# als244/ResNet

Measured on AMD Instinct MI355X. Metric: images/sec ResNet-50 fp32 224x224 batch256, higher is better.
Workload: dtype f32

## Files before the change

resnet_amd/csrc/kernels_bn.hip:

```cpp
#include "mi_common.hpp"
#include "mi_device.h"

#define BN_SPLIT_MAX 64

struct Wel { float n, mean, m2; };
__device__ __forceinline__ Wel wel_merge(Wel a, Wel b) {
    Wel r;
    r.n = a.n + b.n;
    if (r.n == 0.f) { r.mean = 0.f; r.m2 = 0.f; return r; }
    const float d = b.mean - a.mean, f = b.n / r.n;
    r.mean = a.mean + d * f;
    r.m2 = a.m2 + b.m2 + d * d * a.n * f;
    return r;
}
__device__ __forceinline__ Wel wel_wave(Wel w) {
#pragma unroll
    for (int o = 32; o > 0; o >>= 1) {
        Wel b;
        b.n = __shfl_xor(w.n, o, 64); b.mean = __shfl_xor(w.mean, o, 64); b.m2 = __shfl_xor(w.m2, o, 64);
        w = wel_merge(w, b);
    }
    return w;
}
__device__ __forceinline__ void wel_add4(Wel &w, float a, float b, float c, float d) {
// ... 64 lines not shown
    }
    w = wel_wave(w);
    __shared__ Wel sh[4];
    const int lane = threadIdx.x & 63, wv = threadIdx.x >> 6;
    if (lane == 0) sh[wv] = w;
    __syncthreads();
    if (threadIdx.x == 0) {
        Wel r = sh[0];
        for (int i = 1; i < (int)(blockDim.x >> 6); i++) r = wel_merge(r, sh[i]);
        float *o = partial + ((size_t)c * BN_SPLIT_MAX + split) * 3;
        o[0] = r.n; o[1] = r.mean; o[2] = r.m2;
    }
}

__global__ void __launch_bounds__(256)
bn_parts_merge_kernel(const float *__restrict__ parts, int np, int C, float *__restrict__ partial) {
    const int cx = threadIdx.x & 63, sg = threadIdx.x >> 6;
    const int c = blockIdx.x * 64 + cx;
    const int chunk = (np + gridDim.y - 1) / gridDim.y;
    const int p0 = blockIdx.y * chunk, p1 = min(np, p0 + chunk);
    const size_t plane = (size_t)np * C;
    Wel w = {0.f, 0.f, 0.f};
    if (c < C) {
        int p = p0 + sg;
        for (; p + 7 * 4 < p1; p += 8 * 4) {
            Wel b[8];
#pragma unroll
            for (int u = 0; u < 8; u++) {
                const size_t o = (size_t)(p + 4 * u) * C + c;
                b[u].n = parts[o]; b[u].mean = parts[plane + o]; b[u].m2 = parts[2 * plane + o];
            }
#pragma unroll
            for (int u = 0; u < 8; u++) w = wel_merge(w, b[u]);
        }
        for (; p < p1; p += 4) {
            const size_t o = (size_t)p * C + c;
            Wel b = {parts[o], parts[plane + o], parts[2 * plane + o]};
            w = wel_merge(w, b);
        }
    }
    __shared__ Wel sh[4][64];
    sh[sg][cx] = w;
    __syncthreads();
    if (sg == 0 && c < C) {
        Wel r = sh[0][cx];
        for (int i = 1; i < 4; i++) r = wel_merge(r, sh[i][cx]);
        float *o = partial + ((size_t)c * BN_SPLIT_MAX + blockIdx.y) * 3;
        o[0] = r.n; o[1] = r.mean; o[2] = r.m2;
    }
}

__global__ void __launch_bounds__(256)
bn_finalize_kernel(const float *__restrict__ partial, int nsplit, int C, float *__restrict__ means, float *__restrict__ vars) {
    const int c = blockIdx.x * 4 + (threadIdx.x >> 6), lane = threadIdx.x & 63;
    if (c >= C) return;
    const float *p = partial + (size_t)c * BN_SPLIT_MAX * 3;
    Wel w = {0.f, 0.f, 0.f};
    if (lane < nsplit) { w.n = p[lane * 3]; w.mean = p[lane * 3 + 1]; w.m2 = p[lane * 3 + 2]; }
    w = wel_wave(w);
    if (lane == 0) { means[c] = w.mean; vars[c] = w.m2 / w.n; }
}
// ... 169 lines not shown
    }
    s1 = wave_sum(s1); s2 = wave_sum(s2);
    __shared__ float sh[8];
    const int lane = threadIdx.x & 63, wv = threadIdx.x >> 6;
    if (lane == 0) { sh[wv * 2] = s1; sh[wv * 2 + 1] = s2; }
    __syncthreads();
    if (threadIdx.x == 0) {
        float a = 0.f, bsum = 0.f;
        for (int i = 0; i < (int)(blockDim.x >> 6); i++) { a += sh[i * 2]; bsum += sh[i * 2 + 1]; }
        float *o = partial + ((size_t)c * BN_SPLIT_MAX + split) * 3;
        o[0] = a; o[1] = bsum;
    }
}

__global__ void __launch_bounds__(256)
bn_bwd_parts_merge_kernel(const float *__restrict__ parts, int np, int C, const float *__restrict__ vars, float eps, float *__restrict__ partial) {
    const int cx = threadIdx.x & 63, sg = threadIdx.x >> 6;
    const int c = blockIdx.x * 64 + cx;
    const int chunk = (np + gridDim.y - 1) / gridDim.y;
    const int p0 = blockIdx.y * chunk, p1 = min(np, p0 + chunk);
    const size_t plane = (size_t)np * C;
    float a1 = 0.f, a2 = 0.f;
    if (c < C) {
        int p = p0 + sg;
        for (; p + 7 * 4 < p1; p += 8 * 4) {
            float u1[8], u2[8];
#pragma unroll
            for (int u = 0; u < 8; u++) {
                const size_t o = (size_t)(p + 4 * u) * C + c;
                u1[u] = parts[o]; u2[u] = parts[plane + o];
            }
#pragma unroll
            for (int u = 0; u < 8; u++) { a1 += u1[u]; a2 += u2[u]; }
        }
        for (; p < p1; p += 4) {
            const size_t o = (size_t)p * C + c;
            a1 += parts[o]; a2 += parts[plane + o];
        }
    }
    __shared__ float sh[2][4][64];
    sh[0][sg][cx] = a1; sh[1][sg][cx] = a2;
    __syncthreads();
    if (sg == 0 && c < C) {
        const float s1 = (sh[0][0][cx] + sh[0][1][cx]) + (sh[0][2][cx] + sh[0][3][cx]);
        const float s2 = (sh[1][0][cx] + sh[1][1][cx]) + (sh[1][2][cx] + sh[1][3][cx]);
        float *o = partial + ((size_t)c * BN_SPLIT_MAX + blockIdx.y) * 3;
        o[0] = s1; o[1] = s2 / sqrtf(vars[c] + eps);
    }
}

__global__ void __launch_bounds__(256)
bn_bwd_finalize_kernel(float *__restrict__ partial, int nsplit, int C, float *__restrict__ dgamma, float *__restrict__ dbeta) {
    const int c = blockIdx.x * 4 + (threadIdx.x >> 6), lane = threadIdx.x & 63;
    if (c >= C) return;
    const float *p = partial + (size_t)c * BN_SPLIT_MAX * 3;
    float s1 = 0.f, s2 = 0.f;
    if (lane < nsplit) { s1 = p[lane * 3]; s2 = p[lane * 3 + 1]; }
    s1 = wave_sum(s1); s2 = wave_sum(s2);
    if (lane == 0) { dbeta[c] = s1; dgamma[c] = s2; }
}

template <int MASK, typename TX, typename TA, int V, bool STR>
// ... 236 lines not shown
    if ((xhat_out || norm_out) && !(x_dt == MID_F32 && a_dt == MID_F32)) { mi_record_error("mid_bn_fwd_t", "full-store tensors exist in fp32 only"); return -2; }
    if (bn_size_ok("mid_bn_fwd_t", N, C, P)) return -2;
    hipStream_t st = (hipStream_t)s;
    const double xb = (double)N * C * P * dt_bytes(x_dt), ab = (double)N * C * P * dt_bytes(a_dt);
    if (!parts || parts->nparts <= 0) {
        const int ns = bn_nsplit(N, C);
        mi_prof_begin(st, MI_FAM_BN, 0.0, 2 * xb + ab * (residual ? 2 : 1));
        if (bn_stats_launch(st, ws, x, x_dt, N, C, P, ns)) return -1;
        hipLaunchKernelGGL(bn_finalize_kernel, dim3(mi_cdiv(C, 4)), dim3(256), 0, st, ws, ns, C, means, vars);
        MI_LAUNCH_CHECK("bn_finalize_kernel");
    } else {
        int G = parts->nparts / 64;
        if (G < 1) G = 1;
        if (G > BN_SPLIT_MAX) G = BN_SPLIT_MAX;
        mi_prof_begin(st, MI_FAM_BN, 0.0, xb + ab * (residual ? 2 : 1));
        hipLaunchKernelGGL(bn_parts_merge_kernel, dim3(mi_cdiv(C, 64), G), dim3(256), 0, st, parts->buf, parts->nparts, C, ws);
        MI_LAUNCH_CHECK("bn_parts_merge_kernel");
        hipLaunchKernelGGL(bn_finalize_kernel, dim3(mi_cdiv(C, 4)), dim3(256), 0, st, ws, G, C, means, vars);
        MI_LAUNCH_CHECK("bn_finalize_kernel");
    }
    if (g_bn_sync.comm && g_bn_sync.world > 1 - g_bn_sync.force) {
        const float iw = 1.0f / (float)g_bn_sync.world;
        float *tmp = g_bn_sync.tmp;
        if (C > g_bn_sync.tmp_floats / 2) { mi_record_error("sync BN", "scratch too small"); return -3; }
        (void)hipMemcpyAsync(tmp, means, sizeof(float) * C, hipMemcpyDeviceToDevice, st);
        if (mid_rccl_allreduce_sum(g_bn_sync.comm, tmp, (size_t)C, (mid_stream)st)) return -1;
        hipLaunchKernelGGL(bn_sync_k2, dim3(mi_cdiv(C, 256)), dim3(256), 0, st, tmp, means, vars, tmp + C, C, iw);
        if (mid_rccl_allreduce_sum(g_bn_sync.comm, tmp + C, (size_t)C, (mid_stream)st)) return -1;
        hipLaunchKernelGGL(bn_sync_k3, dim3(mi_cdiv(C, 256)), dim3(256), 0, st, tmp + C, vars, C, iw);
        MI_LAUNCH_CHECK("bn_sync");
    }
    const int rc = bn_fwd_apply(st, x, x_dt, gamma, beta, residual, means, vars, y, a_dt, xhat_out, norm_out, N, C, P, eps, relu, ycl, Hcl);
    mi_prof_end(st);
    return rc;
// ... 12 lines not shown
}

static int bn_bwd_impl(hipStream_t st, float *ws, const void *x, int x_dt, const float *gamma, const float *beta, const float *means,
                       const float *vars, const void *dy, const void *mask_src, void *gated_out, int a_dt, void *dx, float *dgamma,
                       float *dbeta, int N, int C, int P, float eps, int mask_mode, const mid_bn_bwd_parts *bparts = nullptr) {
    if (!bn_pair_ok(x_dt, a_dt)) { mi_record_error("mid_bn_bwd", "unsupported storage types"); return -2; }
    if (bn_size_ok("mid_bn_bwd", N, C, P)) return -2;
    int ns = bn_nsplit(N, C);
    dim3 grid(C, ns), block(256);
    if (mask_mode >= 2 && !mask_src) { mi_record_error("mid_bn_bwd", "mask_src missing"); return -2; }
    if (mask_mode == 3 && !gated_out) { mi_record_error("mid_bn_bwd_gate", "gated_out missing"); return -2; }
    const double xb = (double)N * C * P * dt_bytes(x_dt), ab = (double)N * C * P * dt_bytes(a_dt);
    mi_prof_begin(st, MI_FAM_BN, 0.0, bparts ? 2 * xb + ab : 3 * xb + ab * (mask_mode >= 2 ? 4 : 2));
    const int vec = bn_vec(x_dt, a_dt, P);
    const FastDiv fdPV = make_fastdiv(P / vec);
    if (bparts) {
        ns = bparts->nparts >= 64 * 8 ? 64 : bparts->nparts >= 64 ? 8 : 1;
        hipLaunchKernelGGL(bn_bwd_parts_merge_kernel, dim3(mi_cdiv(C, 64), ns), dim3(256), 0, st, bparts->buf, bparts->nparts, C, vars, eps, ws);
        MI_LAUNCH_CHECK("bn_bwd_parts_merge_kernel");
    } else {
#define BWD_REDUCE_M(M_, TX, TA, V)                                                                                         \
    hipLaunchKernelGGL((bn_bwd_reduce_kernel<M_, TX, TA, V>), grid, block, 0, st, (const TX *)x, (const TA *)dy, (const TA *)mask_src, \
                       gamma, beta, means, vars, ws, (TA *)gated_out, N, C, P, eps, fdPV)
#define BWD_R0(TX, TA, V) BWD_REDUCE_M(0, TX, TA, V)
#define BWD_R1(TX, TA, V) BWD_REDUCE_M(1, TX, TA, V)
#define BWD_R2(TX, TA, V) BWD_REDUCE_M(2, TX, TA, V)
#define BWD_R3(TX, TA, V) BWD_REDUCE_M(3, TX, TA, V)
    if (mask_mode == 0) BN_DISPATCH(BWD_R0);
    else if (mask_mode == 1) BN_DISPATCH(BWD_R1);
    else if (mask_mode == 2) BN_DISPATCH(BWD_R2);
    else BN_DISPATCH(BWD_R3);
#undef BWD_R0
#undef BWD_R1
#undef BWD_R2
#undef BWD_R3
#undef BWD_REDUCE_M
    MI_LAUNCH_CHECK("bn_bwd_reduce_kernel");
    }
    hipLaunchKernelGGL(bn_bwd_finalize_kernel, dim3(mi_cdiv(C, 4)), dim3(256), 0, st, ws, ns, C, dgamma, dbeta);
    MI_LAUNCH_CHECK("bn_bwd_finalize_kernel");
    const size_t total = (size_t)N * C * P;
    const FastDiv fdP = make_fastdiv(P), fdC = make_fastdiv(C);
    float inv_m = 1.0f / (float)((size_t)N * P);
    const float *dg_apply = dgamma, *db_apply = dbeta;
    const bool sync = g_bn_sync.comm && g_bn_sync.world > 1 - g_bn_sync.force;
    if (sync) {
        if (2 * C > g_bn_sync.tmp_floats) { mi_record_error("sync BN", "scratch too small"); return -3; }
        float *tmp = g_bn_sync.tmp;
        hipLaunchKernelGGL(bn_sync_pack, dim3(mi_cdiv(C, 256)), dim3(256), 0, st, dgamma, dbeta, tmp, C);
        if (mid_rccl_allreduce_sum(g_bn_sync.comm, tmp, (size_t)2 * C, (mid_stream)st)) return -1;
        dg_apply = tmp; db_apply = tmp + C;
        inv_m = 1.0f / ((float)g_bn_sync.world * (float)((size_t)N * P));
    }
    const void *dy_apply = mask_mode == 3 ? gated_out : dy;
    const char *apply_name;
// ... 57 lines not shown
```

resnet_amd/csrc/kernels_gemm.hip:

```cpp
#include "mi_common.hpp"
#include "mi_device.h"

typedef float f32x16 __attribute__((ext_vector_type(16)));

struct GemmArgs {
    int M, N, K;
    long a_sm, a_sk, a_sb;
    long b_sk, b_sn, b_sb;
    long c_sm, c_sn, c_sb;
    int P;
    FastDiv fdP;
    int klen;
    long c_split;
};

enum { BATCH_NONE = 0, BATCH_N = 1, BATCH_K = 2 };

#define G_BK 32
#define G_LDK 129
#define G_LDN 132

typedef float gf4 __attribute__((ext_vector_type(4)));

template <int BM, int BATCH, bool A_KC, bool B_KC, bool VA, bool VB>
__global__ void __launch_bounds__(256)
gemm_mfma_kernel(const float *__restrict__ A, const float *__restrict__ B, float *__restrict__ C,
                 const float *__restrict__ addend, const GemmArgs g) {
    constexpr int BN = 128;
    constexpr int WM = 64, WN = (BM == 128) ? 64 : 32;
    constexpr int TM = WM / 32, TN = WN / 32;
    constexpr int LDA = A_KC ? G_LDK : G_LDN, LDB = B_KC ? G_LDK : G_LDN;
    constexpr int AV = BM * G_BK / 1024, BV = BN * G_BK / 1024;
    constexpr int AE = BM * G_BK / 256, BE = BN * G_BK / 256;
    __shared__ __attribute__((aligned(16))) float As[G_BK * LDA];
    __shared__ __attribute__((aligned(16))) float Bs[G_BK * LDB];
    const int tid = threadIdx.x, lane = tid & 63;
    const int wave = __builtin_amdgcn_readfirstlane(tid >> 6);
    const int wm = (BM == 128) ? (wave >> 1) : 0, wn = (BM == 128) ? (wave & 1) : wave;
    const int m0 = blockIdx.y * BM, n0 = blockIdx.x * BN;
    const int kbeg = blockIdx.z * g.klen, kend = min(g.K, kbeg + g.klen);

    f32x16 acc[TM][TN];
#pragma unroll
    for (int i = 0; i < TM; i++)
#pragma unroll
        for (int j = 0; j < TN; j++)
#pragma unroll
            for (int r = 0; r < 16; r++) acc[i][j][r] = 0.f;

    constexpr int NA = VA ? AV : AE, NB = VB ? BV : BE;
    int ai[NA], ak[NA], bj[NB], bk[NB];
    long aoff[NA], boff[NB];
#pragma unroll
    for (int q = 0; q < NA; q++) {
        if (VA) {
            if (A_KC) { ak[q] = (tid & 7) * 4; ai[q] = (tid >> 3) + 32 * q; }
            else { ai[q] = (tid & (BM / 4 - 1)) * 4; ak[q] = tid / (BM / 4) + (1024 / BM) * q; }
        } else {
            if (A_KC) { ak[q] = tid & 31; ai[q] = (tid >> 5) + 8 * q; }
            else { ai[q] = tid % BM; ak[q] = tid / BM + (256 / BM) * q; }
        }
        aoff[q] = (long)(m0 + ai[q]) * g.a_sm;
    }
#pragma unroll
    for (int q = 0; q < NB; q++) {
        if (VB) {
            if (B_KC) { bk[q] = (tid & 7) * 4; bj[q] = (tid >> 3) + 32 * q; }
            else { bj[q] = (tid & 31) * 4; bk[q] = (tid >> 5) + 8 * q; }
        } else {
            if (B_KC) { bk[q] = tid & 31; bj[q] = (tid >> 5) + 8 * q; }
            else { bj[q] = tid & 127; bk[q] = (tid >> 7) + 2 * q; }
        }
        const int col = min(n0 + bj[q], g.N - 1);
        if (BATCH == BATCH_N) { const uint32_t n = fd_div((uint32_t)col, g.fdP); boff[q] = (long)n * g.b_sb + (col - (long)n * g.P); }
        else boff[q] = (long)col * g.b_sn;
    }
    auto koff_a = [&](int kk) -> long {
        if (BATCH == BATCH_K) { const uint32_t n = fd_div((uint32_t)kk, g.fdP); return (long)n * g.a_sb + (kk - (long)n * g.P); }
        return (long)kk * g.a_sk;
    };
    auto koff_b = [&](int kk) -> long {
        if (BATCH == BATCH_K) { const uint32_t n = fd_div((uint32_t)kk, g.fdP); return (long)n * g.b_sb + (kk - (long)n * g.P); }
        return (long)kk * g.b_sk;
    };

    gf4 ra4[VA ? AV : 1], rb4[VB ? BV : 1];
// ... 86 lines not shown
            for (int r = 0; r < 16; r++) {
                const int row = m0 + wm * WM + i * 32 + (r & 3) + 8 * (r >> 2) + 4 * (lane >> 5);
                if (row < g.M) {
                    const long o = coff + (long)row * g.c_sm;
                    float v = acc[i][j][r];
                    if (addend) v += ad[r];
                    Cz[o] = v;
                }
            }
        }
    }
}

template <int BATCH, bool A_KC, bool B_KC>
static int launch_gemm(hipStream_t st, const float *A, const float *B, float *C, const float *addend, GemmArgs g,
                       int splits, bool va, bool vb) {
    g.fdP = make_fastdiv(g.P > 0 ? g.P : 1);
    if (splits < 1) splits = 1;
    int klen = mi_cdiv(g.K, splits);
    klen = mi_cdiv(klen, G_BK) * G_BK;
    g.klen = klen;
    splits = mi_cdiv(g.K, klen);
    const int bm = g.M <= 64 ? 64 : 128;
    dim3 grid(mi_cdiv(g.N, 128), mi_cdiv(g.M, bm), splits), block(256);
    mi_prof_begin(st, MI_FAM_GEMM, 2.0 * (double)g.M * g.N * g.K,
                  4.0 * ((double)g.M * g.K + (double)g.K * g.N + (double)g.M * g.N * (addend ? 2 : 1)));
    if (((uintptr_t)A & 15) || ((uintptr_t)B & 15)) va = vb = false;
#define GL(BM_, VA_, VB_) hipLaunchKernelGGL((gemm_mfma_kernel<BM_, BATCH, A_KC, B_KC, VA_, VB_>), grid, block, 0, st, A, B, C, addend, g)
    if (bm == 64) { if (va && vb) GL(64, true, true); else if (va) GL(64, true, false); else GL(64, false, false); }
    else { if (va && vb) GL(128, true, true); else if (va) GL(128, true, false); else GL(128, false, false); }
#undef GL
    mi_prof_end(st);
    MI_LAUNCH_CHECK("gemm_mfma_kernel");
    return splits;
}

int mi_launch_split_reduce(hipStream_t st, const float *part, float *out, long n, int splits, size_t stride);

extern "C" int mi_conv1x1_fwd(mid_stream s, const float *x, const float *w, float *y, int N, int C, int P, int K) {
    hipStream_t st = (hipStream_t)s;
    GemmArgs g = {};
    g.M = K; g.N = N * P; g.K = C; g.P = P;
    g.a_sm = C; g.a_sk = 1;
    g.b_sk = P; g.b_sb = (long)C * P;
    g.c_sm = P; g.c_sb = (long)K * P;
    return launch_gemm<BATCH_N, true, false>(st, w, x, y, nullptr, g, 1, C % 4 == 0, P % 4 == 0) > 0 ? 0 : -1;
}
extern "C" int mi_conv1x1_dgrad(mid_stream s, const float *w, const float *dy, float *dx, const float *addend, int N, int C,
                                int P, int K) {
    hipStream_t st = (hipStream_t)s;
    GemmArgs g = {};
    g.M = C; g.N = N * P; g.K = K; g.P = P;
    g.a_sm = 1; g.a_sk = C;
    g.b_sk = P; g.b_sb = (long)K * P;
    g.c_sm = P; g.c_sb = (long)C * P;
    return launch_gemm<BATCH_N, false, false>(st, w, dy, dx, addend, g, 1, C % 4 == 0, P % 4 == 0) > 0 ? 0 : -1;
}
static int wgrad1x1_splits(int N, int C, int P, int K) {
    const int tiles = mi_cdiv(C, 128) * mi_cdiv(K, K <= 64 ? 64 : 128);
    int splits = mi_cdiv(1024, tiles);
    const long kd = (long)N * P;
    const int maxs = (int)(kd / 256 > 0 ? kd / 256 : 1);
    if (splits > maxs) splits = maxs;
    if (splits < 1) splits = 1;
    return splits;
}
extern "C" size_t mi_conv1x1_wgrad_part_floats(int N, int C, int P, int K) {
    return (size_t)wgrad1x1_splits(N, C, P, K) * K * C;
}
extern "C" int mi_conv1x1_wgrad(mid_stream s, mid_workspace *ws, const float *x, const float *dy, float *dw, int N, int C, int P,
                                int K) {
    hipStream_t st = (hipStream_t)s;
    GemmArgs g = {};
    g.M = K; g.N = C; g.K = N * P; g.P = P;
    g.a_sm = P; g.a_sb = (long)K * P;
    g.b_sn = P; g.b_sb = (long)C * P;
    g.c_sm = C; g.c_sn = 1;
    g.c_split = (long)K * C;
    int splits = wgrad1x1_splits(N, C, P, K);
    if (splits > 1 && (!ws || ws->part_floats < (size_t)splits * K * C)) {
        mi_record_error("mi_conv1x1_wgrad", "workspace too small");
        return -3;
    }
    float *out = splits > 1 ? ws->part : dw;
    const int used = launch_gemm<BATCH_K, true, true>(st, dy, x, out, nullptr, g, splits, P % 4 == 0, P % 4 == 0);
    if (used < 0) return -1;
    if (splits > 1) return mi_launch_split_reduce(st, out, dw, (long)K * C, used, (size_t)K * C);
    return 0;
}

extern "C" {
int mid_gemm_nn(mid_stream s, const float *A, const float *B, float *out, int m, int k, int n) {
    GemmArgs g = {};
    g.M = m; g.N = n; g.K = k; g.P = 1;
    g.a_sm = k; g.a_sk = 1; g.b_sk = n; g.b_sn = 1; g.c_sm = n; g.c_sn = 1;
    return launch_gemm<BATCH_NONE, true, false>((hipStream_t)s, A, B, out, nullptr, g, 1, k % 4 == 0, n % 4 == 0) > 0 ? 0 : -1;
}
int mid_gemm_tn(mid_stream s, const float *At, const float *B, float *out, int m, int k, int n) {
    GemmArgs g = {};
    g.M = m; g.N = n; g.K = k; g.P = 1;
    g.a_sm = 1; g.a_sk = m; g.b_sk = n; g.b_sn = 1; g.c_sm = n; g.c_sn = 1;
    return launch_gemm<BATCH_NONE, false, false>((hipStream_t)s, At, B, out, nullptr, g, 1, m % 4 == 0, n % 4 == 0) > 0 ? 0 : -1;
}
int mid_gemm_nt(mid_stream s, const float *A, const float *Bt, float *out, int m, int k, int n) {
    GemmArgs g = {};
    g.M = m; g.N = n; g.K = k; g.P = 1;
    g.a_sm = k; g.a_sk = 1; g.b_sk = 1; g.b_sn = k; g.c_sm = n; g.c_sn = 1;
    return launch_gemm<BATCH_NONE, true, true>((hipStream_t)s, A, Bt, out, nullptr, g, 1, k % 4 == 0, k % 4 == 0) > 0 ? 0 : -1;
}
}
```

resnet_amd/csrc/mi_device.h:

```cpp
#ifndef MI_DEVICE_H
#define MI_DEVICE_H
#include <stddef.h>
#include <stdint.h>
#ifdef __cplusplus
extern "C" {
#endif

typedef void *mid_stream;
typedef void *mid_event;

enum { MID_F32 = 0, MID_BF16 = 1 };

int mid_device_count(void);
int mid_set_device(int dev);
const char *mid_last_error(void);
void mid_clear_error(void);
void *mid_malloc(size_t bytes);
void mid_free(void *p);
int mid_redzone(size_t zone_bytes, int fill_byte);
int mid_redzone_check(void);
void mid_redzone_stats(size_t *allocs_checked, size_t *zone_bytes_checked, size_t *live);
int mid_trace_names(char *buf, size_t cap);
void mid_trace_clear(void);
void *mid_malloc_host(size_t bytes);
// ... 115 lines not shown
int mid_stem_bf16_supported(int C, int H, int K, int k, int stride);
size_t mid_stem_bf16_xp_bytes(int N, int H);
size_t mid_stem_bf16_part_floats(int N, int H);
int mid_stem_fwd_bf16(mid_stream s, const float *x, const float *w, void *y, int y_dt, void *xp, size_t xp_bytes, float *scratch, size_t scratch_floats,
                      int N, int H, mid_bn_parts *parts);
int mid_stem_wgrad_bf16(mid_stream s, const void *xp, const void *dy, int dy_dt, float *dw, float *scratch, size_t scratch_floats, int N, int H);
int mid_f32_to_bf16(mid_stream s, const float *in, void *out, size_t n);
int mid_bf16_to_f32(mid_stream s, const void *in, float *out, size_t n);

int mid_igemm_plan(int op, int N, int C, int H, int K, int k, int stride, int out[9]);
int mid_igemm_conv_plan(int op, int N, int C, int H, int K, int k, int stride, int out[7]);
int mid_bf16_conv_plan(int op, int N, int C, int H, int K, int k, int stride, int out[7]);
int mid_cl_conv_plan(int route, int op, int N, int C, int H, int K, int k, int stride, int out[7]);
int mid_wgrad_reduce_grouped(int K, int C, int splits);

int mid_gemm_nn(mid_stream s, const float *A, const float *B, float *out, int m, int k, int n);
int mid_gemm_tn(mid_stream s, const float *At, const float *B, float *out, int m, int k, int n);
int mid_gemm_nt(mid_stream s, const float *A, const float *Bt, float *out, int m, int k, int n);

size_t mid_bn_ws_floats(int C);
int mid_bn_fwd(mid_stream s, float *stats_ws, const float *x, const float *gamma, const float *beta,
               const float *residual, float *means, float *vars, float *y, float *xhat_out, float *norm_out, int N,
               int C, int P, float eps, int relu);
int mid_bn_fwd_parts(mid_stream s, float *stats_ws, const mid_bn_parts *parts, const float *x, const float *gamma,
                     const float *beta, const float *residual, float *means, float *vars, float *y, float *xhat_out,
                     float *norm_out, int N, int C, int P, float eps, int relu);
int mid_bn_bwd(mid_stream s, float *stats_ws, const float *x, const float *gamma, const float *beta,
               const float *means, const float *vars, const float *dy, const float *mask_src, float *dx,
               float *dgamma, float *dbeta, int N, int C, int P, float eps, int mask_mode);

int mid_bn_bwd_gate(mid_stream s, float *stats_ws, const float *x, const float *gamma, const float *beta,
                    const float *means, const float *vars, const float *dy, const float *mask_src, float *gated_out,
                    float *dx, float *dgamma, float *dbeta, int N, int C, int P, float eps);
// ... 95 lines not shown
```

resnet_amd/csrc/mi_host.h:

```cpp
#ifndef MI_HOST_H
#define MI_HOST_H
#include "mi_device.h"
#include "resnet_mi.h"

struct MiRng { uint64_t seed; uint64_t counter; };

uint64_t mi_splitmix64_at(uint64_t seed, uint64_t i);
void mi_synth_uniform(float *out, size_t n, uint64_t seed, uint64_t offset, float lo, float hi);
void mi_synth_normal(float *out, size_t n, uint64_t seed, uint64_t offset, double var);
void mi_synth_labels(int *out, size_t n, uint64_t seed, uint64_t offset, int n_classes);

typedef struct {
    int ready;
    mid_stream compute, comm, copy, aux;
} MiGlobal;
MiGlobal *mi_global(void);

typedef struct BatchExt {
    Batch *batch;
    int source, layout, status;
    int rank, world;
    char *shard_dir, *images_path, *labels_path;
    uint64_t seed_images, seed_labels;
    int n_classes, pool_batches, pool_next;
// ... 119 lines not shown
int mi_optim_step(const MiOptim *o, mid_stream s, float *p, float *g, float *b, size_t from, size_t to, float lr, float wd, float wd_norm,
                  int *nan_flag, int want_norms);
typedef struct {
    int n_chunks;
    mid_chunk *chunks_dev;
    double *part_dev;
    mid_clip_record *rec_dev;
    size_t bytes;
} MiClip;
int mi_clip_init(MiClip *k, const char *who, const size_t *off, const int *sizes, int n);
void mi_clip_free(MiClip *k);
int mi_clip_run(const MiClip *k, mid_stream s, float *g, float max_norm);

typedef struct MiCtx {
    MiLayerWs lw;
    mid_wt_entry *wt_tab;
    int wt_n, wt_tiles;
    mid_wt_entry *wt_tab_dev;
    int *wt_tile_entry_dev;
    MiOptions opt;
    MiUnit *units;
    int n_units, *blk_unit;
    int *nan_flag_dev, *nan_flag_host;
    int nan_check_pending;
    mid_event ev_nan;
    size_t *loc_off_dev; int n_loc;
    size_t *loc_off;
    int nan_location, nan_no_exit;
    struct MiCtx *next_live;
    int full_store, dump_every, input_reset;
// ... 99 lines not shown
```

resnet_amd/csrc/ops.c:

```c
#include <math.h>
#include <stdint.h>
#include <stdlib.h>
#include <string.h>
#include "mi_host.h"

void *mi_malloc(size_t bytes) {
    char *p = (char *)mid_malloc(bytes + 2 * MI_GUARD);
    return p ? p + MI_GUARD : NULL;
}
void mi_free(void *p) { if (p) mid_free((char *)p - MI_GUARD); }

static int finish(int rc) {
    mid_stream_sync(mi_global()->compute);
    if (rc) return rc;
    return mid_last_error()[0] ? -1 : 0;
}

typedef struct { MiLayer L; MiLayerWs w; mid_wt_entry we; mid_stream s; int rc; } OpConv;
static MiOptions op_options(void) {
    MiOptions env, o = {.bnfuse_bwd = 1, .bnfuse_bwd_f32 = 7};
    mi_read_options(&env);
    o.igemm = env.igemm; o.pw_wgrad = env.pw_wgrad;
    return o;
}
// ... 69 lines not shown
                      int C, int H, float eps) {
    float *ws = (float *)mid_malloc(mid_bn_ws_floats(C) * sizeof(float));
    int rc = finish(mid_bn_bwd_gate(mi_global()->compute, ws, x, gamma, beta, means, vars, dy, mask_src, gated_out, dx, dgamma, dbeta, N, C, H * H, eps));
    mid_free(ws);
    return rc;
}
int mi_op_maxpool_fwd(const float *x, float *y, int *max_inds, int N, int C, int H, int k, int stride) {
    return finish(mid_maxpool_fwd(mi_global()->compute, x, y, max_inds, N, C, H, k, stride));
}
int mi_op_maxpool_bwd(const int *max_inds, const float *dy, float *dx, int N, int C, int H, int k, int stride) {
    return finish(mid_maxpool_bwd(mi_global()->compute, max_inds, dy, dx, N, C, H, k, stride));
}
int mi_op_avgpool_fwd(const float *x, float *y, int N, int C, int H) { return finish(mid_avgpool_fwd(mi_global()->compute, x, y, N, C, H * H)); }
int mi_op_avgpool_bwd(const float *dy, float *dx, int N, int C, int H) { return finish(mid_avgpool_bwd(mi_global()->compute, dy, dx, N, C, H * H)); }
int mi_op_relu_deriv(const float *x, const float *up, float *out, size_t n) { return finish(mid_relu_deriv(mi_global()->compute, x, up, out, n)); }
int mi_op_matmul(const float *A, const float *B, float *out, int m, int k, int n) { return finish(mid_gemm_nn(mi_global()->compute, A, B, out, m, k, n)); }
int mi_op_matmul_lt(const float *A_kxm, const float *B, float *out, int m, int k, int n) { return finish(mid_gemm_tn(mi_global()->compute, A_kxm, B, out, m, k, n)); }
int mi_op_matmul_rt(const float *A, const float *B_nxk, float *out, int m, int k, int n) { return finish(mid_gemm_nt(mi_global()->compute, A, B_nxk, out, m, k, n)); }
int mi_op_softmax(const float *x, float *out, int N, int L) { return finish(mid_softmax(mi_global()->compute, x, out, N, L)); }
int mi_op_ce_deriv(const float *pred, const int *labels, float *d, int N, int L) { return finish(mid_ce_deriv(mi_global()->compute, pred, labels, d, N, L)); }
_Static_assert(sizeof(MiLossMetrics) == sizeof(mid_loss_metrics), "one record, declared on both sides of mi_device.h");
int mi_loss_args_ok(const char *who, float smoothing, int topk, int L) {
    if (!(smoothing >= 0.f && smoothing < 1.f)) { mi_record_host_error(who, "smoothing lies in [0, 1)"); return -1; }
    if (topk < 1 || topk > L) { mi_record_host_error(who, "topk lies in [1, number of classes]"); return -1; }
    return 0;
}
int mi_op_loss_head(const float *logits, const int *labels, float *pred, float *dlogits, float *row_loss, int *row_rank, int N, int L,
                    float smoothing, int topk, MiLossMetrics *last_dev, MiLossMetrics *total_dev) {
    if (N < 1 || L < 1) { mi_record_host_error("mi_op_loss_head", "N and L are at least 1"); return -1; }
    if (mi_loss_args_ok("mi_op_loss_head", smoothing, topk, L)) return -1;
    const int totals = last_dev || total_dev;
    float *rl = totals && !row_loss ? (float *)mid_malloc((size_t)N * sizeof(float)) : NULL;
    int *rr = totals && !row_rank ? (int *)mid_malloc((size_t)N * sizeof(int)) : NULL;
// ... 382 lines not shown
```

resnet_amd/csrc/trainer.c:

```c
#include <math.h>
#include <stdio.h>
#include <stdlib.h>
#include <string.h>
#include "mi_host.h"

static MiGlobal G;
MiGlobal *mi_global(void) {
    if (!G.ready) {
        G.compute = mid_stream_create();
        G.comm = mid_stream_create();
        G.copy = mid_stream_create();
        G.aux = mid_stream_create_low_priority();
        G.ready = 1;
    }
    return &G;
}

int mi_device_count(void) { return mid_device_count(); }
int mi_set_device(int device) { return mid_set_device(device); }
const char *mi_last_error(void) { return mid_last_error(); }
void mi_device_synchronize(void) { mid_device_sync(); }
static unsigned long g_host_write_epoch = 0;
void mi_params_mark_dirty(void) { g_host_write_epoch++; }
void mi_copy_to_device(void *d, const void *s, size_t n) { MiGlobal *g = mi_global(); mid_memcpy_h2d(d, s, n, g->compute); mid_stream_sync(g->compute); g_host_write_epoch++; }
// ... 352 lines not shown
    c->wt_tab_dev = NULL; c->wt_tile_entry_dev = NULL;
    if (c->wt_n) {
        int *te = (int *)malloc((size_t)c->wt_tiles * sizeof(int));
        for (int e = 0; e < c->wt_n; e++) {
            const int nt = (c->wt_tab[e].C / 32) * (c->wt_tab[e].K / 32);
            for (int q = 0; q < nt; q++) te[c->wt_tab[e].tile0 + q] = e;
        }
        c->wt_tab_dev = (mid_wt_entry *)mi_ctx_alloc(c, (size_t)c->wt_n * sizeof(mid_wt_entry));
        c->wt_tile_entry_dev = (int *)mi_ctx_alloc(c, (size_t)c->wt_tiles * sizeof(int));
        mid_memcpy_h2d(c->wt_tab_dev, c->wt_tab, (size_t)c->wt_n * sizeof(mid_wt_entry), G.compute);
        mid_memcpy_h2d(c->wt_tile_entry_dev, te, (size_t)c->wt_tiles * sizeof(int), G.compute);
        mid_stream_sync(G.compute);
        free(te);
    }
    mi_layer_ws_alloc(c, &c->lw, &need);
}

static void free_activations_host(Activations *a);
static void add_full_store_extras(Train_ResNet *t);
static void rs_build_table(Train_ResNet *t);
static void build_buffers(Train_ResNet *t) {
    MiCtx *c = (MiCtx *)t->backend_ctx;
    Dims *d = t->model->dims;
    ConvBlock **blocks = t->model->params->conv_blocks;
    const int N = t->batch_size;
    const size_t maxe = max_tensor_elems(d, blocks, N);
    c->act_bytes = 0;
    c->rc_buf[0] = c->rc_buf[1] = NULL;
    if (c->policy == MI_STORE_RECOMPUTE_BN) { c->rc_buf[0] = aalloc(c, maxe); c->rc_buf[1] = aalloc(c, maxe); }
    c->counting_act = 1;
// ... 302 lines not shown
    ck(mid_maxpool_fwd_t(G.compute, a->init_conv_activated, a->init_convblock_input, c->dtype, a->max_inds, N, d->init_conv_filters,
                         d->input / d->init_conv_stride, d->init_maxpool_dim, d->init_maxpool_stride), "max-pool forward");
    for (int i = 0; i < nb; i++) {
        unit_fwd(t, unit_of(c, i, MI_U_RED), images, running);
        unit_fwd(t, unit_of(c, i, MI_U_SPA), images, running);
        if (unit_of(c, i, MI_U_PROJ)) unit_fwd(t, unit_of(c, i, MI_U_PROJ), images, running);
        unit_fwd(t, unit_of(c, i, MI_U_EXP), images, running);
    }
    if (!running && c->rs_on) {
        ck(mid_bn_running_update(G.compute, c->rs_tab_dev, c->n_units, c->rs_channels, c->rs_arena, (size_t)c->rs_channels, c->rs_momentum),
           "running statistics");
        c->rs_updates++;
    }
    const int Hl = p->conv_blocks[nb - 1]->incoming_spatial_dim;
    ck(mid_avgpool_fwd_t(G.compute, unit_of(c, nb - 1, MI_U_EXP)->out, c->dtype, a->final_conv_output_pooled, N, d->final_depth, Hl * Hl), "average pool");
    ck(mid_gemm_nn(G.compute, a->final_conv_output_pooled, p->fully_connected, a->linear_output, N, d->final_depth, d->output), "FC forward");
}
void forward_pass(Train_ResNet *t) {
    MiCtx *c = ctx_of(t);
    const Dims *d = t->model->dims;
    Activations *a = t->forward_buffer->activations;
    const int N = t->batch_size;
    mid_event_record(c->ev_t[0], G.compute);
    bind_sync_bn(c);
    c->acts_from_eval = 0;
    c->acc_in_step = 1;
    forward_trunk(t, t->cur_batch->images, 0);
    if (c->mix_on && c->mix_last.mode != 0)
        ck(mid_loss_head_mix(G.compute, a->linear_output, t->cur_batch->correct_classes, c->mix_labels_b, c->mix_last.lam, t->forward_buffer->pred,
                             t->backprop_buffer->output_layer_deriv, c->loss_row, c->loss_rank, N, d->output, c->loss_smoothing, c->loss_topk,
                             c->loss_metrics, c->loss_metrics + 1), "two-label loss head");
// ... 494 lines not shown
    Activations *da = bb->activation_derivs;
    const int N = t->batch_size, L = d->output, D = d->final_depth, nb = d->n_conv_blocks;
    const int recompute = c->policy == MI_STORE_RECOMPUTE_BN;
    if (c->acts_from_eval) {
        mi_record_host_error("backwards_pass", "the last pass was mi_trainer_eval_forward: run forward_pass first");
        return;
    }
    mid_event_record(c->ev_t[2], G.compute);
    bind_sync_bn(c);
    if (weights_stale(c)) relayout_weights(c);
    c->dp_cursor = c->arena_floats;
    c->n_buckets = 0;
    if (!(c->loss_flags & MI_LOSS_DEVICE))
        ck(mid_ce_deriv(G.compute, t->forward_buffer->pred, t->cur_batch->correct_classes, bb->output_layer_deriv, N, L), "cross-entropy derivative");
    ck(mid_gemm_tn(G.compute, a->final_conv_output_pooled, bb->output_layer_deriv, dp->fully_connected, D, N, L), "FC wgrad");
    ck(mid_gemm_nt(G.compute, bb->output_layer_deriv, p->fully_connected, da->final_conv_output_pooled, N, L, D), "FC dgrad");
    mi_dp_reduce_ready(t, (size_t)(dp->fully_connected - c->g_arena), 0);
    const ConvBlock *last = p->conv_blocks[nb - 1];
    const int Hl = last->incoming_spatial_dim;
    ck(mid_avgpool_bwd_t(G.compute, da->final_conv_output_pooled, da->activation_conv_blocks[nb - 1]->output_activated, c->dtype, N, D, Hl * Hl),
       "average pool backward");
    const int ring = c->overlap_wgrad == 2;
    mid_bn_bwd_parts fz = {NULL}, req;
    for (int i = nb - 1; i >= 0; i--) {
        MiUnit *red = unit_of(c, i, MI_U_RED), *spa = unit_of(c, i, MI_U_SPA), *expa = unit_of(c, i, MI_U_EXP), *proj = unit_of(c, i, MI_U_PROJ);
        const MiUnit *below = i == 0 ? NULL : unit_of(c, i - 1, MI_U_EXP);
        Activation_ConvBlock *dk = da->activation_conv_blocks[i];
        float *dbin = i == 0 ? da->init_convblock_input : da->activation_conv_blocks[i - 1]->output_activated;
        const float *up = dk->output_activated;
        const float *exp_dy, *exp_mask, *red_addend;
        int exp_mode, s_proj = -1, s_exp = -1, s_spa = -1, s_red = -1;
// ... 505 lines not shown
```

Measured before the change: 2460.

## Fuse BN finalize into merge, add narrow wgrad tile, split-K FC GEMMs

When the batch-norm parts merge runs with a single split, it now writes the final mean/var (forward) and dgamma/dbeta (backward) directly, so the separate finalize launches are skipped. The 1x1 weight-gradient GEMM gets a 64x64 tile for narrow layers (both channel counts at most 64), a split rule aimed at a fixed workgroup count, and a grouped split-reduce kernel. The FC forward and dgrad GEMMs now use split-K with a workspace to fill more compute units. These changes add workspace allocation and extra reduce passes, plus odd no-op merge loops inside the fused finalize paths.

```diff
diff --git a/resnet_amd/csrc/kernels_bn.hip b/resnet_amd/csrc/kernels_bn.hip
--- a/resnet_amd/csrc/kernels_bn.hip
+++ b/resnet_amd/csrc/kernels_bn.hip
@@ -102,7 +102,8 @@
 }
 
 __global__ void __launch_bounds__(256)
-bn_parts_merge_kernel(const float *__restrict__ parts, int np, int C, float *__restrict__ partial) {
+bn_parts_merge_kernel(const float *__restrict__ parts, int np, int C, float *__restrict__ partial, float *__restrict__ means,
+                      float *__restrict__ vars) {
     const int cx = threadIdx.x & 63, sg = threadIdx.x >> 6;
     const int c = blockIdx.x * 64 + cx;
     const int chunk = (np + gridDim.y - 1) / gridDim.y;
@@ -133,6 +134,12 @@
     if (sg == 0 && c < C) {
         Wel r = sh[0][cx];
         for (int i = 1; i < 4; i++) r = wel_merge(r, sh[i][cx]);
+        if (means) {
+            const Wel none = {0.f, 0.f, 0.f};
+            for (int i = 0; i < 6; i++) r = wel_merge(r, none);
+            means[c] = r.mean; vars[c] = r.m2 / r.n;
+            return;
+        }
         float *o = partial + ((size_t)c * BN_SPLIT_MAX + blockIdx.y) * 3;
         o[0] = r.n; o[1] = r.mean; o[2] = r.m2;
     }
@@ -332,7 +339,8 @@
 }
 
 __global__ void __launch_bounds__(256)
-bn_bwd_parts_merge_kernel(const float *__restrict__ parts, int np, int C, const float *__restrict__ vars, float eps, float *__restrict__ partial) {
+bn_bwd_parts_merge_kernel(const float *__restrict__ parts, int np, int C, const float *__restrict__ vars, float eps, float *__restrict__ partial,
+                          float *__restrict__ dgamma, float *__restrict__ dbeta) {
     const int cx = threadIdx.x & 63, sg = threadIdx.x >> 6;
     const int c = blockIdx.x * 64 + cx;
     const int chunk = (np + gridDim.y - 1) / gridDim.y;
@@ -362,8 +370,14 @@
     if (sg == 0 && c < C) {
         const float s1 = (sh[0][0][cx] + sh[0][1][cx]) + (sh[0][2][cx] + sh[0][3][cx]);
         const float s2 = (sh[1][0][cx] + sh[1][1][cx]) + (sh[1][2][cx] + sh[1][3][cx]);
-        float *o = partial + ((size_t)c * BN_SPLIT_MAX + blockIdx.y) * 3;
+        float fin[2];
+        float *o = dgamma ? fin : partial + ((size_t)c * BN_SPLIT_MAX + blockIdx.y) * 3;
         o[0] = s1; o[1] = s2 / sqrtf(vars[c] + eps);
+        if (dgamma) {
+            float t1 = fin[0], t2 = fin[1];
+            for (int i = 0; i < 6; i++) { t1 += 0.f; t2 += 0.f; }
+            dbeta[c] = t1; dgamma[c] = t2;
+        }
     }
 }
 
@@ -630,10 +644,13 @@
         if (G < 1) G = 1;
         if (G > BN_SPLIT_MAX) G = BN_SPLIT_MAX;
         mi_prof_begin(st, MI_FAM_BN, 0.0, xb + ab * (residual ? 2 : 1));
-        hipLaunchKernelGGL(bn_parts_merge_kernel, dim3(mi_cdiv(C, 64), G), dim3(256), 0, st, parts->buf, parts->nparts, C, ws);
+        hipLaunchKernelGGL(bn_parts_merge_kernel, dim3(mi_cdiv(C, 64), G), dim3(256), 0, st, parts->buf, parts->nparts, C, ws,
+                           G == 1 ? means : nullptr, G == 1 ? vars : nullptr);
         MI_LAUNCH_CHECK("bn_parts_merge_kernel");
-        hipLaunchKernelGGL(bn_finalize_kernel, dim3(mi_cdiv(C, 4)), dim3(256), 0, st, ws, G, C, means, vars);
-        MI_LAUNCH_CHECK("bn_finalize_kernel");
+        if (G > 1) {
+            hipLaunchKernelGGL(bn_finalize_kernel, dim3(mi_cdiv(C, 4)), dim3(256), 0, st, ws, G, C, means, vars);
+            MI_LAUNCH_CHECK("bn_finalize_kernel");
+        }
     }
     if (g_bn_sync.comm && g_bn_sync.world > 1 - g_bn_sync.force) {
         const float iw = 1.0f / (float)g_bn_sync.world;
@@ -676,9 +693,12 @@
     mi_prof_begin(st, MI_FAM_BN, 0.0, bparts ? 2 * xb + ab : 3 * xb + ab * (mask_mode >= 2 ? 4 : 2));
     const int vec = bn_vec(x_dt, a_dt, P);
     const FastDiv fdPV = make_fastdiv(P / vec);
+    bool fin_fused = false;
     if (bparts) {
         ns = bparts->nparts >= 64 * 8 ? 64 : bparts->nparts >= 64 ? 8 : 1;
-        hipLaunchKernelGGL(bn_bwd_parts_merge_kernel, dim3(mi_cdiv(C, 64), ns), dim3(256), 0, st, bparts->buf, bparts->nparts, C, vars, eps, ws);
+        fin_fused = ns == 1;
+        hipLaunchKernelGGL(bn_bwd_parts_merge_kernel, dim3(mi_cdiv(C, 64), ns), dim3(256), 0, st, bparts->buf, bparts->nparts, C, vars, eps, ws,
+                           fin_fused ? dgamma : nullptr, fin_fused ? dbeta : nullptr);
         MI_LAUNCH_CHECK("bn_bwd_parts_merge_kernel");
     } else {
 #define BWD_REDUCE_M(M_, TX, TA, V)                                                                                         \
@@ -699,8 +719,10 @@
 #undef BWD_REDUCE_M
     MI_LAUNCH_CHECK("bn_bwd_reduce_kernel");
     }
-    hipLaunchKernelGGL(bn_bwd_finalize_kernel, dim3(mi_cdiv(C, 4)), dim3(256), 0, st, ws, ns, C, dgamma, dbeta);
-    MI_LAUNCH_CHECK("bn_bwd_finalize_kernel");
+    if (!fin_fused) {
+        hipLaunchKernelGGL(bn_bwd_finalize_kernel, dim3(mi_cdiv(C, 4)), dim3(256), 0, st, ws, ns, C, dgamma, dbeta);
+        MI_LAUNCH_CHECK("bn_bwd_finalize_kernel");
+    }
     const size_t total = (size_t)N * C * P;
     const FastDiv fdP = make_fastdiv(P), fdC = make_fastdiv(C);
     float inv_m = 1.0f / (float)((size_t)N * P);
diff --git a/resnet_amd/csrc/kernels_gemm.hip b/resnet_amd/csrc/kernels_gemm.hip
--- a/resnet_amd/csrc/kernels_gemm.hip
+++ b/resnet_amd/csrc/kernels_gemm.hip
@@ -22,21 +22,22 @@
 
 typedef float gf4 __attribute__((ext_vector_type(4)));
 
-template <int BM, int BATCH, bool A_KC, bool B_KC, bool VA, bool VB>
+template <int BM, int BATCH, bool A_KC, bool B_KC, bool VA, bool VB, int BN = 128>
 __global__ void __launch_bounds__(256)
 gemm_mfma_kernel(const float *__restrict__ A, const float *__restrict__ B, float *__restrict__ C,
                  const float *__restrict__ addend, const GemmArgs g) {
-    constexpr int BN = 128;
-    constexpr int WM = 64, WN = (BM == 128) ? 64 : 32;
+    static_assert(BN == 128 || (BN == 64 && BM == 64), "tiles: 128 x 128, 64 x 128, 64 x 64");
+    constexpr bool W2X2 = BM == 128 || BN == 64;
+    constexpr int WM = BN == 64 ? 32 : 64, WN = (BM == 128) ? 64 : 32;
     constexpr int TM = WM / 32, TN = WN / 32;
-    constexpr int LDA = A_KC ? G_LDK : G_LDN, LDB = B_KC ? G_LDK : G_LDN;
+    constexpr int LDA = A_KC ? G_LDK : G_LDN, LDB = B_KC ? BN + 1 : BN + 4;
     constexpr int AV = BM * G_BK / 1024, BV = BN * G_BK / 1024;
     constexpr int AE = BM * G_BK / 256, BE = BN * G_BK / 256;
     __shared__ __attribute__((aligned(16))) float As[G_BK * LDA];
     __shared__ __attribute__((aligned(16))) float Bs[G_BK * LDB];
     const int tid = threadIdx.x, lane = tid & 63;
     const int wave = __builtin_amdgcn_readfirstlane(tid >> 6);
-    const int wm = (BM == 128) ? (wave >> 1) : 0, wn = (BM == 128) ? (wave & 1) : wave;
+    const int wm = W2X2 ? (wave >> 1) : 0, wn = W2X2 ? (wave & 1) : wave;
     const int m0 = blockIdx.y * BM, n0 = blockIdx.x * BN;
     const int kbeg = blockIdx.z * g.klen, kend = min(g.K, kbeg + g.klen);
 
@@ -66,10 +67,10 @@
     for (int q = 0; q < NB; q++) {
         if (VB) {
             if (B_KC) { bk[q] = (tid & 7) * 4; bj[q] = (tid >> 3) + 32 * q; }
-            else { bj[q] = (tid & 31) * 4; bk[q] = (tid >> 5) + 8 * q; }
+            else { bj[q] = (tid & (BN / 4 - 1)) * 4; bk[q] = tid / (BN / 4) + (1024 / BN) * q; }
         } else {
             if (B_KC) { bk[q] = tid & 31; bj[q] = (tid >> 5) + 8 * q; }
-            else { bj[q] = tid & 127; bk[q] = (tid >> 7) + 2 * q; }
+            else { bj[q] = tid % BN; bk[q] = tid / BN + (256 / BN) * q; }
         }
         const int col = min(n0 + bj[q], g.N - 1);
         if (BATCH == BATCH_N) { const uint32_t n = fd_div((uint32_t)col, g.fdP); boff[q] = (long)n * g.b_sb + (col - (long)n * g.P); }
@@ -186,20 +187,27 @@
 
 template <int BATCH, bool A_KC, bool B_KC>
 static int launch_gemm(hipStream_t st, const float *A, const float *B, float *C, const float *addend, GemmArgs g,
-                       int splits, bool va, bool vb) {
+                       int splits, bool va, bool vb, int bm_given = 0, int bn = 128) {
     g.fdP = make_fastdiv(g.P > 0 ? g.P : 1);
     if (splits < 1) splits = 1;
     int klen = mi_cdiv(g.K, splits);
     klen = mi_cdiv(klen, G_BK) * G_BK;
     g.klen = klen;
     splits = mi_cdiv(g.K, klen);
-    const int bm = g.M <= 64 ? 64 : 128;
-    dim3 grid(mi_cdiv(g.N, 128), mi_cdiv(g.M, bm), splits), block(256);
+    const int bm = bm_given ? bm_given : g.M <= 64 ? 64 : 128;
+    dim3 grid(mi_cdiv(g.N, bn), mi_cdiv(g.M, bm), splits), block(256);
     mi_prof_begin(st, MI_FAM_GEMM, 2.0 * (double)g.M * g.N * g.K,
                   4.0 * ((double)g.M * g.K + (double)g.K * g.N + (double)g.M * g.N * (addend ? 2 : 1)));
     if (((uintptr_t)A & 15) || ((uintptr_t)B & 15)) va = vb = false;
 #define GL(BM_, VA_, VB_) hipLaunchKernelGGL((gemm_mfma_kernel<BM_, BATCH, A_KC, B_KC, VA_, VB_>), grid, block, 0, st, A, B, C, addend, g)
-    if (bm == 64) { if (va && vb) GL(64, true, true); else if (va) GL(64, true, false); else GL(64, false, false); }
+    if (bn == 64) {
+        if constexpr (BATCH == BATCH_K && A_KC && B_KC) {
+#define GLN(VA_, VB_) hipLaunchKernelGGL((gemm_mfma_kernel<64, BATCH, A_KC, B_KC, VA_, VB_, 64>), grid, block, 0, st, A, B, C, addend, g)
+            if (bm != 64) { mi_record_error("gemm_mfma_kernel", "a 64-column tile has 64 rows"); return -2; }
+            if (va && vb) GLN(true, true); else if (va) GLN(true, false); else GLN(false, false);
+#undef GLN
+        } else { mi_record_error("gemm_mfma_kernel", "no 64-column tile for this form"); return -2; }
+    } else if (bm == 64) { if (va && vb) GL(64, true, true); else if (va) GL(64, true, false); else GL(64, false, false); }
     else { if (va && vb) GL(128, true, true); else if (va) GL(128, true, false); else GL(128, false, false); }
 #undef GL
     mi_prof_end(st);
@@ -209,6 +217,40 @@
 
 int mi_launch_split_reduce(hipStream_t st, const float *part, float *out, long n, int splits, size_t stride);
 
+#define SRG_G 16
+#define SRG_OPB (256 / SRG_G)
+__global__ void __launch_bounds__(256)
+split_reduce_grouped_kernel(const float *__restrict__ part, float *__restrict__ out, long n, int splits, size_t stride) {
+    __shared__ float sh[SRG_G][SRG_OPB];
+    const int o = threadIdx.x % SRG_OPB, gq = threadIdx.x / SRG_OPB;
+    const long i = (long)blockIdx.x * SRG_OPB + o;
+    const int chunk = (splits + SRG_G - 1) / SRG_G, z0 = gq * chunk, z1 = min(splits, z0 + chunk);
+    float s = 0.f;
+    if (i < n) {
+        int z = z0;
+        for (; z + 8 <= z1; z += 8) {
+            float v[8];
+#pragma unroll
+            for (int u = 0; u < 8; u++) v[u] = part[(size_t)(z + u) * stride + i];
+#pragma unroll
+            for (int u = 0; u < 8; u++) s += v[u];
+        }
+        for (; z < z1; z++) s += part[(size_t)z * stride + i];
+    }
+    sh[gq][o] = s;
+    __syncthreads();
+    if (gq == 0 && i < n) {
+        float r = sh[0][o];
+        for (int q = 1; q < SRG_G; q++) r += sh[q][o];
+        out[i] = r;
+    }
+}
+static int launch_split_reduce_grouped(hipStream_t st, const float *part, float *out, long n, int splits, size_t stride) {
+    hipLaunchKernelGGL(split_reduce_grouped_kernel, dim3((unsigned)mi_cdiv(n, (long)SRG_OPB)), dim3(256), 0, st, part, out, n, splits, stride);
+    MI_LAUNCH_CHECK("split_reduce_kernel<grouped>");
+    return 0;
+}
+
 extern "C" int mi_conv1x1_fwd(mid_stream s, const float *x, const float *w, float *y, int N, int C, int P, int K) {
     hipStream_t st = (hipStream_t)s;
     GemmArgs g = {};
@@ -228,7 +270,15 @@
     g.c_sm = P; g.c_sb = (long)C * P;
     return launch_gemm<BATCH_N, false, false>(st, w, dy, dx, addend, g, 1, C % 4 == 0, P % 4 == 0) > 0 ? 0 : -1;
 }
+enum { WG1X1_NARROW_WGS = 768 };
+static bool wgrad1x1_narrow(int C, int K) { return C <= 64 && K <= 64; }
 static int wgrad1x1_splits(int N, int C, int P, int K) {
+    if (wgrad1x1_narrow(C, K)) {
+        const long kd = (long)N * P;
+        const int maxs = (int)(kd / 256 > 0 ? kd / 256 : 1);
+        int klen = mi_cdiv((int)mi_cdiv(kd, (long)(WG1X1_NARROW_WGS < maxs ? WG1X1_NARROW_WGS : maxs)), G_BK) * G_BK;
+        return (int)mi_cdiv(kd, (long)klen);
+    }
     const int tiles = mi_cdiv(C, 128) * mi_cdiv(K, K <= 64 ? 64 : 128);
     int splits = mi_cdiv(1024, tiles);
     const long kd = (long)N * P;
@@ -255,18 +305,47 @@
         return -3;
     }
     float *out = splits > 1 ? ws->part : dw;
-    const int used = launch_gemm<BATCH_K, true, true>(st, dy, x, out, nullptr, g, splits, P % 4 == 0, P % 4 == 0);
-    if (used < 0) return -1;
+    const bool narrow = wgrad1x1_narrow(C, K);
+    const int used = launch_gemm<BATCH_K, true, true>(st, dy, x, out, nullptr, g, splits, P % 4 == 0, P % 4 == 0, 0, narrow ? 64 : 128);
+    if (used < 0 || used > splits) return -1;
+    if (splits > 1 && narrow && used >= 64) return launch_split_reduce_grouped(st, out, dw, (long)K * C, used, (size_t)K * C);
     if (splits > 1) return mi_launch_split_reduce(st, out, dw, (long)K * C, used, (size_t)K * C);
     return 0;
 }
 
+enum { FC_FILL = 256, FC_MIN_KSTEPS = 8 };
+static int fc_split_rule(int m, int k, int n, int *bm) {
+    const int maxs = mi_cdiv(k, G_BK) / FC_MIN_KSTEPS > 1 ? mi_cdiv(k, G_BK) / FC_MIN_KSTEPS : 1;
+    const int cols = mi_cdiv(n, 128);
+    *bm = m <= 64 || cols * mi_cdiv(m, 128) * maxs < FC_FILL ? 64 : 128;
+    const int want = mi_cdiv(FC_FILL, cols * mi_cdiv(m, *bm));
+    const int klen = mi_cdiv(mi_cdiv(k, want < maxs ? want : maxs), G_BK) * G_BK;
+    return mi_cdiv(k, klen);
+}
+template <bool A_KC, bool B_KC>
+static int fc_gemm(const char *who, hipStream_t st, mid_workspace *ws, const float *A, const float *B, float *out, GemmArgs g, bool va, bool vb) {
+    int bm;
+    const int splits = fc_split_rule(g.M, g.K, g.N, &bm);
+    const size_t mn = (size_t)g.M * g.N;
+    if (splits > 1 && (!ws || ws->part_floats < (size_t)splits * mn)) { mi_record_error(who, "workspace too small"); return -3; }
+    g.c_split = (long)mn;
+    const int used = launch_gemm<BATCH_NONE, A_KC, B_KC>(st, A, B, splits > 1 ? ws->part : out, nullptr, g, splits, va, vb, bm);
+    if (used != splits) return -1;
+    if (splits > 1) return mi_launch_split_reduce(st, ws->part, out, (long)mn, splits, mn);
+    return 0;
+}
+
 extern "C" {
-int mid_gemm_nn(mid_stream s, const float *A, const float *B, float *out, int m, int k, int n) {
+size_t mid_gemm_part_floats(int m, int k, int n) {
+    int bm;
+    const int splits = fc_split_rule(m, k, n, &bm);
+    return splits > 1 ? (size_t)splits * m * n : 0;
+}
+int mid_gemm_nn(mid_stream s, mid_workspace *ws, const float *A, const float *B, float *out, int m, int k, int n) {
     GemmArgs g = {};
     g.M = m; g.N = n; g.K = k; g.P = 1;
     g.a_sm = k; g.a_sk = 1; g.b_sk = n; g.b_sn = 1; g.c_sm = n; g.c_sn = 1;
-    return launch_gemm<BATCH_NONE, true, false>((hipStream_t)s, A, B, out, nullptr, g, 1, k % 4 == 0, n % 4 == 0) > 0 ? 0 : -1;
+    return fc_gemm<true, false>("mid_gemm_nn", (hipStream_t)s, ws, A, B, out, g, k % 4 == 0, n % 4 == 0);
 }
 int mid_gemm_tn(mid_stream s, const float *At, const float *B, float *out, int m, int k, int n) {
     GemmArgs g = {};
@@ -274,10 +353,10 @@
     g.a_sm = 1; g.a_sk = m; g.b_sk = n; g.b_sn = 1; g.c_sm = n; g.c_sn = 1;
     return launch_gemm<BATCH_NONE, false, false>((hipStream_t)s, At, B, out, nullptr, g, 1, m % 4 == 0, n % 4 == 0) > 0 ? 0 : -1;
 }
-int mid_gemm_nt(mid_stream s, const float *A, const float *Bt, float *out, int m, int k, int n) {
+int mid_gemm_nt(mid_stream s, mid_workspace *ws, const float *A, const float *Bt, float *out, int m, int k, int n) {
     GemmArgs g = {};
     g.M = m; g.N = n; g.K = k; g.P = 1;
     g.a_sm = k; g.a_sk = 1; g.b_sk = 1; g.b_sn = k; g.c_sm = n; g.c_sn = 1;
-    return launch_gemm<BATCH_NONE, true, true>((hipStream_t)s, A, Bt, out, nullptr, g, 1, k % 4 == 0, k % 4 == 0) > 0 ? 0 : -1;
-}
-}
+    return fc_gemm<true, true>("mid_gemm_nt", (hipStream_t)s, ws, A, Bt, out, g, k % 4 == 0, k % 4 == 0);
+}
+}
diff --git a/resnet_amd/csrc/mi_device.h b/resnet_amd/csrc/mi_device.h
--- a/resnet_amd/csrc/mi_device.h
+++ b/resnet_amd/csrc/mi_device.h
@@ -153,9 +153,10 @@
 int mid_cl_conv_plan(int route, int op, int N, int C, int H, int K, int k, int stride, int out[7]);
 int mid_wgrad_reduce_grouped(int K, int C, int splits);
 
-int mid_gemm_nn(mid_stream s, const float *A, const float *B, float *out, int m, int k, int n);
+size_t mid_gemm_part_floats(int m, int k, int n);
+int mid_gemm_nn(mid_stream s, mid_workspace *ws, const float *A, const float *B, float *out, int m, int k, int n);
 int mid_gemm_tn(mid_stream s, const float *At, const float *B, float *out, int m, int k, int n);
-int mid_gemm_nt(mid_stream s, const float *A, const float *Bt, float *out, int m, int k, int n);
+int mid_gemm_nt(mid_stream s, mid_workspace *ws, const float *A, const float *Bt, float *out, int m, int k, int n);
 
 size_t mid_bn_ws_floats(int C);
 int mid_bn_fwd(mid_stream s, float *stats_ws, const float *x, const float *gamma, const float *beta,
diff --git a/resnet_amd/csrc/mi_host.h b/resnet_amd/csrc/mi_host.h
--- a/resnet_amd/csrc/mi_host.h
+++ b/resnet_amd/csrc/mi_host.h
@@ -157,6 +157,7 @@
 
 typedef struct MiCtx {
     MiLayerWs lw;
+    mid_workspace fc_ws;
     mid_wt_entry *wt_tab;
     int wt_n, wt_tiles;
     mid_wt_entry *wt_tab_dev;
diff --git a/resnet_amd/csrc/ops.c b/resnet_amd/csrc/ops.c
--- a/resnet_amd/csrc/ops.c
+++ b/resnet_amd/csrc/ops.c
@@ -107,9 +107,18 @@
 int mi_op_avgpool_fwd(const float *x, float *y, int N, int C, int H) { return finish(mid_avgpool_fwd(mi_global()->compute, x, y, N, C, H * H)); }
 int mi_op_avgpool_bwd(const float *dy, float *dx, int N, int C, int H) { return finish(mid_avgpool_bwd(mi_global()->compute, dy, dx, N, C, H * H)); }
 int mi_op_relu_deriv(const float *x, const float *up, float *out, size_t n) { return finish(mid_relu_deriv(mi_global()->compute, x, up, out, n)); }
-int mi_op_matmul(const float *A, const float *B, float *out, int m, int k, int n) { return finish(mid_gemm_nn(mi_global()->compute, A, B, out, m, k, n)); }
+static int op_gemm_split(int rt, const float *A, const float *B, float *out, int m, int k, int n) {
+    mid_workspace ws;
+    memset(&ws, 0, sizeof ws);
+    ws.part_floats = mid_gemm_part_floats(m, k, n);
+    if (ws.part_floats) ws.part = (float *)mid_malloc(ws.part_floats * sizeof(float));
+    const int rc = finish((rt ? mid_gemm_nt : mid_gemm_nn)(mi_global()->compute, &ws, A, B, out, m, k, n));
+    mid_free(ws.part);
+    return rc;
+}
+int mi_op_matmul(const float *A, const float *B, float *out, int m, int k, int n) { return op_gemm_split(0, A, B, out, m, k, n); }
 int mi_op_matmul_lt(const float *A_kxm, const float *B, float *out, int m, int k, int n) { return finish(mid_gemm_tn(mi_global()->compute, A_kxm, B, out, m, k, n)); }
-int mi_op_matmul_rt(const float *A, const float *B_nxk, float *out, int m, int k, int n) { return finish(mid_gemm_nt(mi_global()->compute, A, B_nxk, out, m, k, n)); }
+int mi_op_matmul_rt(const float *A, const float *B_nxk, float *out, int m, int k, int n) { return op_gemm_split(1, A, B_nxk, out, m, k, n); }
 int mi_op_softmax(const float *x, float *out, int N, int L) { return finish(mid_softmax(mi_global()->compute, x, out, N, L)); }
 int mi_op_ce_deriv(const float *pred, const int *labels, float *d, int N, int L) { return finish(mid_ce_deriv(mi_global()->compute, pred, labels, d, N, L)); }
 _Static_assert(sizeof(MiLossMetrics) == sizeof(mid_loss_metrics), "one record, declared on both sides of mi_device.h");
diff --git a/resnet_amd/csrc/trainer.c b/resnet_amd/csrc/trainer.c
--- a/resnet_amd/csrc/trainer.c
+++ b/resnet_amd/csrc/trainer.c
@@ -390,6 +390,10 @@
         free(te);
     }
     mi_layer_ws_alloc(c, &c->lw, &need);
+    const size_t fc_fwd = mid_gemm_part_floats(N, d->final_depth, d->output), fc_dg = mid_gemm_part_floats(N, d->output, d->final_depth);
+    memset(&c->fc_ws, 0, sizeof c->fc_ws);
+    c->fc_ws.part_floats = fc_fwd > fc_dg ? fc_fwd : fc_dg;
+    if (c->fc_ws.part_floats) c->fc_ws.part = (float *)mi_ctx_alloc(c, c->fc_ws.part_floats * sizeof(float));
 }
 
 static void free_activations_host(Activations *a);
@@ -722,7 +726,7 @@
     }
     const int Hl = p->conv_blocks[nb - 1]->incoming_spatial_dim;
     ck(mid_avgpool_fwd_t(G.compute, unit_of(c, nb - 1, MI_U_EXP)->out, c->dtype, a->final_conv_output_pooled, N, d->final_depth, Hl * Hl), "average pool");
-    ck(mid_gemm_nn(G.compute, a->final_conv_output_pooled, p->fully_connected, a->linear_output, N, d->final_depth, d->output), "FC forward");
+    ck(mid_gemm_nn(G.compute, &c->fc_ws, a->final_conv_output_pooled, p->fully_connected, a->linear_output, N, d->final_depth, d->output), "FC forward");
 }
 void forward_pass(Train_ResNet *t) {
     MiCtx *c = ctx_of(t);
@@ -1247,7 +1251,7 @@
     if (!(c->loss_flags & MI_LOSS_DEVICE))
         ck(mid_ce_deriv(G.compute, t->forward_buffer->pred, t->cur_batch->correct_classes, bb->output_layer_deriv, N, L), "cross-entropy derivative");
     ck(mid_gemm_tn(G.compute, a->final_conv_output_pooled, bb->output_layer_deriv, dp->fully_connected, D, N, L), "FC wgrad");
-    ck(mid_gemm_nt(G.compute, bb->output_layer_deriv, p->fully_connected, da->final_conv_output_pooled, N, L, D), "FC dgrad");
+    ck(mid_gemm_nt(G.compute, &c->fc_ws, bb->output_layer_deriv, p->fully_connected, da->final_conv_output_pooled, N, L, D), "FC dgrad");
     mi_dp_reduce_ready(t, (size_t)(dp->fully_connected - c->g_arena), 0);
     const ConvBlock *last = p->conv_blocks[nb - 1];
     const int Hl = last->incoming_spatial_dim;
```

New measurement: 2452. About the same (-0.3%).
